# sergcpp/Ray

Hardware: AMD Instinct MI355X
Metric: Msamples/sec (W*H*spp/time) (higher is better)
Workload: dtype f32

## Files before the change

ray_amd/csrc/kernels.hip.h:

```cpp
#pragma once

#include <hip/hip_runtime.h>

#ifdef RT_PROFILE_TRACE
namespace rt {
__device__ unsigned long long g_prof_acc[32];
__shared__ unsigned long long s_prof_last;
__shared__ unsigned long long s_prof_acc[32];
__device__ __forceinline__ void prof_mark(const int k) {
    const unsigned long long mask = __ballot(1);
    if (int(__lane_id()) == __ffsll((long long)mask) - 1) {
        const unsigned long long t = __builtin_readcyclecounter();
        s_prof_acc[k] += t - s_prof_last;
        s_prof_last = t;
    }
}
__device__ __forceinline__ void prof_wait(float4 &a, float4 &b, float4 &c, float4 &d) {
    asm volatile("s_waitcnt vmcnt(0)" : "+v"(a.x), "+v"(b.x), "+v"(c.x), "+v"(d.x));
}
}
#define RT_PROF_T(k) ::rt::prof_mark(k);
#define RT_PROF_LANES(k)                                                                                                \
    {                                                                                                                   \
        const unsigned long long m_ = __ballot(1);                                                                      \
// ... 363 lines not shown
        AccumPixel st = load_accum_pixel(idx, px.full, px.half, px.required_samples);
        const float4 b0 = px.base_color[idx], d0 = px.depth_normals[idx];
        f4 base = {b0.x, b0.y, b0.z, b0.w}, dn = {d0.x, d0.y, d0.z, d0.w};
        AccumParams pl = p;
        for (int k = 0; k < layer_count; ++k) {
            const uint32_t off = layer_offset_xy(layers, uint32_t(layer_base + k));
            const size_t vidx = (size_t(off & 0xffffu) + size_t(y)) * pitch + size_t(off >> 16) + size_t(x);
            fold_layer(pl, per_layer.l[k], px.temp + vidx, px.aux_base_layers + vidx, px.aux_dn_layers + vidx, st, base, dn);
        }
        px.base_color[idx] = mkfloat4(base.x, base.y, base.z, base.w);
        px.depth_normals[idx] = mkfloat4(dn.x, dn.y, dn.z, dn.w);
        store_accum_pixel(pl, idx, st, px.variance + idx, px.full, px.half, px.raw, px.final_, px.required_samples);
    }
}

constexpr int ACCUM_STRIP = 128;
constexpr int ACCUM_SEG_COLS = 8;
constexpr int ACCUM_LOADS = ACCUM_STRIP * ACCUM_SEG_COLS / 256;
static_assert(ACCUM_LOADS * 256 == ACCUM_STRIP * ACCUM_SEG_COLS, "a segment is a whole number of rounds of the block");
__global__ void __launch_bounds__(256) k_accumulate_interleaved(const AccumParams p, const PixelBuffers px, const Layering layers,
                                                               const AccumLayers per_layer, const int layer_base, const int layer_count,
                                                               const int seg_cols) {
    extern __shared__ float4 accum_lds[];
    const int stage = ACCUM_STRIP * seg_cols + 1;
    float4 *const s_temp = accum_lds, *const s_base = accum_lds + stage, *const s_dn = accum_lds + 2 * stage;
    const size_t pitch = size_t(virtual_width(layers));
    const int cols = layers.cols, rows = layers.rows;
    const int strips_x = (p.rect[2] + ACCUM_STRIP - 1) / ACCUM_STRIP, n_strips = strips_x * p.rect[3];
    const int tid = int(threadIdx.x);
    for (int strip = blockIdx.x; strip < n_strips; strip += gridDim.x) {
        const int y = p.rect[1] + strip / strips_x, x0 = p.rect[0] + (strip % strips_x) * ACCUM_STRIP;
        const int np = min(ACCUM_STRIP, p.rect[0] + p.rect[2] - x0);
        const int x = x0 + tid;
        const bool mine = tid < np && pixel_owned(p.shard, p.w, x, y);
        if (!__syncthreads_or(mine ? 1 : 0)) {
            continue;
        }
        const int idx = y * p.w + (mine ? x : x0);
        AccumPixel st = {};
        f4 base = {}, dn = {};
        if (mine) {
            st = load_accum_pixel(idx, px.full, px.half, px.required_samples);
            const float4 b0 = px.base_color[idx], d0 = px.depth_normals[idx];
            base = {b0.x, b0.y, b0.z, b0.w}, dn = {d0.x, d0.y, d0.z, d0.w};
        }
        AccumParams pl = p;
        for (int l0 = layer_base, end = layer_base + layer_count; l0 < end;) {
            const int vr = l0 / cols, c0 = l0 - vr * cols;
            const int len = min(min(seg_cols, cols - c0), end - l0);
            const size_t row0 = (size_t(y) * size_t(rows) + size_t(vr)) * pitch + size_t(x0) * size_t(cols) + size_t(c0);
            const uint32_t rcp = layer_rcp(uint32_t(len));
            const int swizzle = len == 8 ? 7 : 0;
            const int n_elems = np * len;
#pragma unroll
            for (int u = 0; u < ACCUM_LOADS; ++u) {
                const int e = tid + u * 256, e_in = min(e, n_elems - 1);
                const int j = int(div_by_rcp(uint32_t(e_in), rcp));
                const size_t g = row0 + size_t(j) * size_t(cols) + size_t(e_in - j * len);
                const float4 t = px.temp[g], b = px.aux_base_layers[g], d = px.aux_dn_layers[g];
                const int e_out = e < n_elems ? j * len + ((e_in - j * len) ^ (j & swizzle)) : stage - 1;
                s_temp[e_out] = t, s_base[e_out] = b, s_dn[e_out] = d;
            }
            __syncthreads();
            if (mine) {
                for (int k = 0; k < len; ++k) {
                    const int e = tid * len + (k ^ (tid & swizzle));
                    fold_layer(pl, per_layer.l[l0 - layer_base + k], s_temp + e, s_base + e, s_dn + e, st, base, dn);
                }
            }
            __syncthreads();
            l0 += len;
        }
        if (mine) {
            px.base_color[idx] = mkfloat4(base.x, base.y, base.z, base.w);
            px.depth_normals[idx] = mkfloat4(dn.x, dn.y, dn.z, dn.w);
            store_accum_pixel(pl, idx, st, px.variance + idx, px.full, px.half, px.raw, px.final_, px.required_samples);
        }
    }
}

__global__ void __launch_bounds__(256) k_retonemap(const AccumParams p, const PixelBuffers px, const int h) {
    const int n = p.w * h;
    for (int i = blockIdx.x * blockDim.x + threadIdx.x; i < n; i += gridDim.x * blockDim.x) {
        const float4 ff = px.full[i];
        px.raw[i] = ff;
        const f4 c = tonemap(p, f4{ff.x, ff.y, ff.z, ff.w});
// ... 175 lines not shown
```

ray_amd/csrc/rayhip_ctx.hip.h:

```cpp
#pragma once

namespace {
thread_local std::string g_err;

int fail(const char *fmt, ...) {
    char buf[1024];
    va_list vl;
    va_start(vl, fmt);
    vsnprintf(buf, sizeof(buf), fmt, vl);
    va_end(vl);
    g_err = buf;
    return 1;
}

#define HIP_TRY(expr)                                                                                                  \
    do {                                                                                                               \
        const hipError_t _e = (expr);                                                                                  \
        if (_e != hipSuccess) {                                                                                        \
            return fail("%s failed: %s (%s:%d)", #expr, hipGetErrorString(_e), __FILE__, __LINE__);                    \
        }                                                                                                              \
    } while (0)

constexpr int MAX_BOUNCE_SLOTS = 130;

// ... 228 lines not shown
    }
    DevBuf skin_stage;
    DevBuf skin_palettes;
    DevBuf skin_counters;
    DevBuf instance_stage, instance_args, instance_counters;
    bool adaptive_dirty = false;
    int lut_transform = 0, lut_dims = 0;
    PixelBuffers px = {};

    DevBuf ray_planes[2][5], hit_planes[2], shadow_planes[3], deferred_planes[2], point_planes[7], nee_index;
    PointSoA points = {};
    DevBuf pick_plane, record_ray_planes[4];
    RaySoA record_rays = {};
    bool notex_kernels = true;
    bool pick_lds = true;
    bool shade_lds_tables = true;
    uint32_t shade_lds_materials_max = 0xffffffffu, shade_lds_instances_max = 0xffffffffu;
    bool surface_park = true;
    uint32_t shade_tag = 0;
    uint32_t next_shade_tag() {
        if (++shade_tag == 0u) {
            (void)hipMemsetAsync(pick_plane.p, 0, pick_plane.bytes, stream);
            shade_tag = 1u;
        }
        return shade_tag;
    }
    int shade_split = 29;
    RaySoA rays[2] = {};
    HitSoA hits = {};
    ShadowSoA shadow = {};
// ... 483 lines not shown
        c->layer_layout = atoi(e) != 0 ? 1 : 0;
    }
    if (const char *e = getenv("RAYHIP_SORT_KEY")) {
        c->sort_key_mode = std::max(0, std::min(3, atoi(e)));
    }
    if (const char *e = getenv("RAYHIP_SHADE_SPLIT")) {
        c->shade_split = atoi(e) & 31;
        c->shade_form_auto = false;
    }
    if (const char *e = getenv("RAYHIP_NOTEX_KERNELS")) {
        c->notex_kernels = atoi(e) != 0;
    }
    if (const char *e = getenv("RAYHIP_PICK_LDS")) {
        c->pick_lds = atoi(e) != 0;
    }
    if (const char *e = getenv("RAYHIP_SURFACE_PARK")) {
        c->surface_park = atoi(e) != 0;
    }
    if (const char *e = getenv("RAYHIP_SHADE_LDS_TABLES")) {
        c->shade_lds_tables = atoi(e) != 0;
    }
    if (const char *e = getenv("RAYHIP_SHADE_LDS_MATERIALS_MAX")) {
        c->shade_lds_materials_max = uint32_t(std::max(0, atoi(e)));
    }
    if (const char *e = getenv("RAYHIP_SHADE_LDS_INSTANCES_MAX")) {
        c->shade_lds_instances_max = uint32_t(std::max(0, atoi(e)));
    }
    if (c->stack_spill.alloc(size_t(c->grid_waves) * std::max(STACK_SPILL_DEPTH * WAVE, POOL_SLAB_WORDS) * sizeof(uint32_t)) ||
        (c->trace.overlap_shadow && c->stack_spill2.alloc(size_t(c->grid_waves) * size_t(STACK_SPILL_DEPTH * WAVE) * sizeof(uint32_t)))) {
        delete c;
// ... 196 lines not shown
```

ray_amd/csrc/rayhip_render.hip.h:

```cpp
#pragma once

static bool pass_fits(const rayhip_ctx *c, const int rect[4], int n) {
    const Layering L = make_layering(c->w, c->h, n, c->layer_layout);
    const size_t vbytes = size_t(c->w) * size_t(c->h) * size_t(L.cols) * size_t(layer_rows(L)) * 16u;
    return vbytes <= c->px_temp.bytes && (n <= 1 || (vbytes <= c->px_aux_base.bytes && vbytes <= c->px_aux_dn.bytes)) &&
           pass_slots(c, c->w, c->h, rect[2], rect[3], n) + size_t(WAVE) * QUEUE_MAX_STRIPES <= c->slots_cap;
}
static bool rect_inside(const rayhip_ctx *c, const int rect[4]) {
    return rect[0] >= 0 && rect[1] >= 0 && rect[2] > 0 && rect[3] > 0 && rect[0] <= c->w - rect[2] && rect[1] <= c->h - rect[3];
}
static int ensure_pass(rayhip_ctx *c, const int rect[4], int n) {
    if (!rect_inside(c, rect)) {
        return fail("rect outside the frame");
    }
    if (!pass_fits(c, rect, n)) {
        HIP_TRY(hipStreamSynchronize(c->stream));
        if (alloc_frame(c, c->w, c->h, n)) {
            return 1;
        }
    }
    return 0;
}

static void launch_shade(rayhip_ctx *c, const rayhip_camera &cam, int iteration, int bounce, int cur, size_t nslots, uint32_t stripes,
                         int gtrace, int vw, float mix_factor, const Layering &layers, bool plain_ior = false, bool sized = false, int split = -1) {
    ShadeLaunch a;
    a.sc = c->sc;
    a.sp = make_shade_params(cam, iteration, bounce);
    a.sp.plain_ior = plain_ior ? 1u : 0u;
    a.rays_in = c->rays[cur], a.rays_out = c->rays[cur ^ 1];
    a.hits = c->hits, a.shadow = c->shadow, a.deferred = c->deferred, a.points = c->points;
    a.in = c->ray_queue(bounce, nslots, stripes), a.pts = c->point_queue(bounce, nslots, stripes);
    a.out_rays = c->ray_queue(bounce + 1, nslots, stripes), a.out_shadow = c->shadow_queue(bounce, nslots, stripes);
    a.out_deferred = c->deferred_queue(bounce, nslots, stripes), a.nee = c->nee_queue(bounce, nslots, stripes);
    a.out_sky = c->sky_queue(bounce, nslots, stripes), a.sky_index = c->sky_index.as<uint32_t>();
    a.px = c->px, a.layers = layers, a.vw = vw, a.mix_factor = mix_factor;
    a.bounce = bounce, a.grid = gtrace, a.split = split >= 0 ? split : c->shade_split, a.stream = c->stream;
    a.picks = c->pick_plane.as<float4>(), a.record_rays = c->record_rays, a.tag = c->next_shade_tag();
    a.pick_lds = c->pick_lds, a.surface_park = c->surface_park;
    a.lds_tables = c->shade_lds_tables, a.n_materials = c->geometry.materials, a.n_instances = c->instances_count;
    a.lds_materials_max = c->shade_lds_materials_max, a.lds_instances_max = c->shade_lds_instances_max;
    a.no_textures = c->textures_count == 0 && c->notex_kernels;
    if (sized) {
        a.expect[EXPECT_RAYS] = bounce == 0 ? uint32_t(nslots / WAVE + stripes) : c->expect_chunks(bounce, 0, nslots, stripes);
        a.expect[EXPECT_POINTS] = c->expect_chunks(bounce, 3, nslots, stripes), a.expect[EXPECT_LIT] = c->expect_chunks(bounce, 4, nslots, stripes);
        a.expect[EXPECT_DEFERRED] = c->expect_chunks(bounce, 2, nslots, stripes), a.expect[EXPECT_SKY] = c->expect_chunks(bounce, 5, nslots, stripes);
        a.chunks_per_block = c->chunks_per_block;
        a.work = c->next_work(), a.chunks = uint32_t((nslots + WAVE - 1) / WAVE + stripes), a.dyn_mult = c->dyn_mult;
    }
    shade::launch(a);
}

static int render_pass(rayhip_ctx *c, const rayhip_camera *cam, const int rect[4], int iteration, int count_iterations,
                       uint32_t flags, rayhip_stats *stats) {
// ... 38 lines not shown
        return fail("internal: pass of %d iterations exceeds the allocated wavefront state", count_iterations);
    }
    const int gw = c->grid_waves;
    const int gtrace = int(std::min<size_t>(size_t(gw), nslots / WAVE));
    unsigned long long *tc = c->trav_counters.as<unsigned long long>();
    uint32_t *spill = c->stack_spill.as<uint32_t>();
    const TraceParams tp = make_trace_params(*cam, c->sc.tlas_root, iteration);

    const uint32_t stripes = sort_rays ? 1u : QUEUE_MAX_STRIPES;
    if (c->census_on && c->census_pending && hipEventQuery(c->census_event) == hipSuccess) {
        const double inv = c->census_slots ? 1.0 / double(c->census_slots) : 0.0;
        for (int k = 0; k < c->census_bounces * rayhip_ctx::QUEUES_PER_BOUNCE; ++k) {
            c->census[size_t(k)] = float(double(c->census_host[k]) * inv);
        }
        c->census_valid = true, c->census_pending = false;
    }
    int bounce_now = 0;
    auto dyn_grid = [&](int resident, uint32_t expect) {
        const size_t chunks = expect ? size_t(expect) : (nslots + WAVE - 1) / WAVE + stripes;
        return int(std::max<size_t>(1, std::min<size_t>({size_t(gw), size_t(std::max(resident, 1)) * size_t(c->dyn_mult), chunks})));
    };
    auto static_grid = [&](int full, int resident, uint32_t expect) {
        if (!expect) {
            return full;
        }
        const uint32_t want = std::max(std::min(expect, uint32_t(std::max(resident, 1))), expect / uint32_t(c->chunks_per_block));
        return int(std::min<uint32_t>(uint32_t(full), std::max(want, 1u)));
    };
    auto trace_closest = [&](const RaySoA &r, const RayQueue &q, int init_hits) {
        const ClosestForm form = closest_form(c->trace, c->wide, c->direct(), init_hits ? TraceRole::Secondary : TraceRole::Primary, flags);
// ... 145 lines not shown
        side_pending = false;
    }
    if (tm.mark(-1, -1)) {
        return 1;
    }
    AccumParams ap = make_accum_params(*cam, c->w, rect, iteration, c->shard);
    ap.lut = c->tonemap_lut.as<uint32_t>(), ap.lut_dims = c->lut_dims;
    for (int base = 0; base < count_iterations; base += MAX_BATCH) {
        const int n = std::min(MAX_BATCH, count_iterations - base);
        AccumLayers per_layer = {};
        for (int k = 0; k < n; ++k) {
            const AccumParams al = make_accum_params(*cam, c->w, rect, iteration + base + k, c->shard);
            per_layer.l[k] = AccumLayer{al.iteration, al.mix_factor, al.half_mix_factor, al.is_class_a, al.variance_threshold};
        }
        if (layers.interleaved && layers.count > 1) {
            const int seg_cols = std::min(layers.cols, ACCUM_SEG_COLS);
            const size_t strips = size_t((rect[2] + ACCUM_STRIP - 1) / ACCUM_STRIP) * size_t(rect[3]);
            const size_t lds = 3u * (size_t(ACCUM_STRIP) * size_t(seg_cols) + 1u) * sizeof(float4);
            k_accumulate_interleaved<<<grid_for(c, strips * 256u, 256), 256, lds, s>>>(ap, c->px, layers, per_layer, base, n, seg_cols);
        } else {
            k_accumulate<<<grid_for(c, npix, 256), 256, 0, s>>>(ap, c->px, layers, per_layer, base, n);
        }
    }
    if (c->census_on && !count && !count_wide) {
        const int queues = (max_depth + 1) * rayhip_ctx::QUEUES_PER_BOUNCE;
        k_queue_totals<<<queues, WAVE, 0, s>>>(c->counters.as<uint32_t>(), c->census_dev);
        HIP_TRY(hipEventRecord(c->census_event, s));
        c->census_pending = true, c->census_bounces = max_depth + 1, c->census_slots = nslots;
    }
    HIP_TRY(hipGetLastError());
    if (tm.mark(-1, -1)) {
        return 1;
    }
    if (stats) {
// ... 71 lines not shown
```

ray_amd/csrc/shade_kernels.hip:

```cpp
#include <hip/hip_runtime.h>

#include <algorithm>
#include <map>
#include <mutex>
#include <utility>

#ifdef RT_PROFILE_SHADE
namespace rt {
__device__ unsigned long long g_prof_shade[64];
}
#define RT_PROF_SHADE_LANES(k)                                                                                          \
    {                                                                                                                   \
        const unsigned long long m_ = __ballot(1);                                                                      \
        if (int(__lane_id()) == __ffsll((long long)m_) - 1) {                                                           \
            atomicAdd(&::rt::g_prof_shade[k], (unsigned long long)__popcll(m_));                                        \
            atomicAdd(&::rt::g_prof_shade[(k) + 1], 1ull);                                                              \
        }                                                                                                               \
    }
#endif

#include "shade_launch.h"

namespace rt {
namespace shade {
// ... 586 lines not shown
        }
        Scatter sct;
        sct.has_next = sct.has_shadow = false;
        if (continues) {
            ray.o = pt.P, ray.pdf = 0.0f;
            scatter_stage<false, true>(sc, tb, spl, ray, pt, no_light_pick(), sct, &ahead);
            sct.next.xy = xy;
        }
        const uint32_t n_slot = out_rays.alloc(stripe, sct.has_next);
        if (sct.has_next) {
            store_ray(rays_out, n_slot, sct.next, sp.plain_ior == 0u);
        }
    }
}

__global__ void __launch_bounds__(WAVE) k_shade_emissive(const SceneView sc, const ShadeParams sp, const RaySoA rays_in, const HitSoA hits,
                                                        const DeferredSoA deferred, const RayQueue queue, const PixelBuffers px,
                                                        const int img_w) {
    const uint32_t lane = threadIdx.x;
    const uint32_t n_live_chunks = queue.live_chunks();
    ChunkWalk walk(n_live_chunks);
    for (uint32_t c; walk.next(c);) {
        uint32_t stripe, slot0, n_live;
        if (!queue.chunk(c, stripe, slot0, n_live) || lane >= n_live) {
            continue;
        }
        const float4 a = deferred.a[slot0 + lane], b = deferred.b[slot0 + lane];
        const uint32_t i = float_as_uint(a.x), tri = float_as_uint(a.y), material = float_as_uint(a.z);
        const float4 o = rays_in.o_pdf[i], d = rays_in.d_cw[i], throughput = rays_in.c_cs[i];
        const uint32_t xy = rays_in.xy_depth[i].x;
        const Hit hit = load_hit(hits, i);
        const f3 origin = {o.x, o.y, o.z}, dir = {d.x, d.y, d.z};
        const float mis = emissive_hit_mis_weight(sc, origin, dir, origin + hit.t * dir, hit.t, o.w, tri, &sc.mesh_instances[hit.obj_index]);
        ShadeResult res;
        res.col = emissive_hit_radiance(sp, a.w, mis, sc.materials[material].tangent_rotation_or_strength, f3{b.x, b.y, b.z},
                                        f3{throughput.x, throughput.y, throughput.z});
        add_secondary_pixel(res, xy, img_w, px.temp);
    }
}
// ... 9 lines not shown
        if (!queue.chunk(c, stripe, slot0, n_live) || lane >= n_live) {
            continue;
        }
        const uint32_t i = sky_index[slot0 + lane];
        Ray ray = load_ray(rays_in, i, sp.plain_ior == 0u);
        const Hit hit = load_hit(hits, i);
        const uint32_t xy = ray.xy, layer = xy_layer(xy, layers);
        const ShadeParams spl = layer_params(sp, layer);
        ray.xy = xy_real(xy, layers, layer);
        add_sky_pixel(shade_sky_ray(sc, ray, hit, spl.iteration, int(spl.ps.max_total_depth), spl.limits[0]), xy, img_w, px.temp);
    }
}



static int resident_blocks(const void *kernel) {
    static std::mutex mu;
    static std::map<std::pair<int, const void *>, int> cache;
    int dev = 0;
    (void)hipGetDevice(&dev);
    std::lock_guard<std::mutex> lock(mu);
    const auto key = std::make_pair(dev, kernel);
    const auto it = cache.find(key);
    if (it != cache.end()) {
        return it->second;
    }
    int per_cu = 0, cus = 0;
    if (hipOccupancyMaxActiveBlocksPerMultiprocessor(&per_cu, kernel, WAVE, 0) != hipSuccess || per_cu <= 0 ||
        hipDeviceGetAttribute(&cus, hipDeviceAttributeMultiprocessorCount, dev) != hipSuccess) {
        per_cu = 0;
    }
    return cache[key] = per_cu * cus;
}

void launch(const ShadeLaunch &a) {
    hipStream_t s = a.stream;
    const int g = a.grid;
    auto sized = [&](auto kernel, const uint32_t expect, const int cap) {
        int grid = std::min(g, cap);
        if (expect != 0u && a.chunks_per_block > 0) {
            const int resident = std::max(1, resident_blocks(reinterpret_cast<const void *>(kernel)));
            const uint32_t want = std::max(std::min(expect, uint32_t(resident)), expect / uint32_t(a.chunks_per_block));
            grid = int(std::min<uint32_t>(uint32_t(grid), std::max(want, 1u)));
        }
        return grid;
    };
    const int all = 1 << 30;
    if ((a.split & 16) != 0) {
        const bool lights = a.sc.light_cwnodes_count != 0;
        if (lights) {
            const uint32_t lds_nodes = (a.pick_lds && a.sc.light_cwnodes_count <= PICK_LDS_MAX_NODES) ? a.sc.light_cwnodes_count : 0u;
            auto go = [&](auto kernel, auto kernel_wave) {
                int grid = sized(kernel_wave, a.expect[EXPECT_RAYS], all);
                if (a.work) {
                    const int resident = std::max(1, resident_blocks(reinterpret_cast<const void *>(kernel_wave))) * std::max(1, a.dyn_mult);
                    const uint32_t bound = a.expect[EXPECT_RAYS] != 0u ? a.expect[EXPECT_RAYS] : a.chunks;
                    grid = int(std::max<uint32_t>(1u, std::min<uint32_t>({uint32_t(g), uint32_t(resident), std::max(bound, 1u)})));
                }
                if (lds_nodes != 0u) {
                    kernel<<<(grid + PICK_BLOCK_WAVES - 1) / PICK_BLOCK_WAVES, PICK_BLOCK_WAVES * WAVE, size_t(lds_nodes) * LIGHT_CHILDREN_STRIDE * sizeof(float4), s>>>(
                        a.sc, a.sp, a.rays_in, a.hits, a.in, a.picks, a.tag, a.layers, a.work, lds_nodes);
                } else {
                    kernel_wave<<<grid, WAVE, 0, s>>>(a.sc, a.sp, a.rays_in, a.hits, a.in, a.picks, a.tag, a.layers, a.work, 0u);
                }
            };
            a.work ? go(k_light_pick_first<true, true>, k_light_pick_first<true, false>) : go(k_light_pick_first<false, true>, k_light_pick_first<false, false>);
        }
#define RT_FUSED(...) k_surface_scatter<__VA_ARGS__><<<sized(k_surface_scatter<__VA_ARGS__>, a.expect[EXPECT_RAYS], all), WAVE, 0, s>>>( \
        a.sc, a.sp, a.rays_in, a.hits, a.in, a.picks, a.tag, a.points, a.record_rays, a.nee, a.rays_out, a.out_rays, a.deferred, a.out_deferred, a.px, a.vw, \
        a.mix_factor, a.layers, a.sky_index, a.out_sky, a.n_materials, a.n_instances)
// ... 15 lines not shown
        } else if (sky_scene) {
            RT_FUSED(false, true);
        } else if (a.no_textures) {
            if (lds_tables) {
                park ? RT_FUSED(false, false, false, true, true) : RT_FUSED(false, false, false, false, true);
            } else {
                park ? RT_FUSED(false, false, false, true) : RT_FUSED(false, false, false);
            }
        } else {
            RT_FUSED(false, false);
        }
#undef RT_FUSED
        if (sky_scene) {
            k_shade_sky<<<sized(k_shade_sky, a.expect[EXPECT_SKY], 4096), WAVE, 0, s>>>(a.sc, a.sp, a.rays_in, a.hits, a.sky_index, a.out_sky, a.px, a.vw, a.layers);
        }
        k_shade_emissive<<<sized(k_shade_emissive, a.expect[EXPECT_DEFERRED], 2048), WAVE, 0, s>>>(a.sc, a.sp, a.rays_in, a.hits, a.deferred, a.out_deferred, a.px, a.vw);
        if (lights) {
            auto nee = [&](auto kernel) {
                kernel<<<sized(kernel, a.expect[EXPECT_LIT], all), WAVE, 0, s>>>(
                    a.sc, a.sp, a.record_rays, a.points, a.nee, a.rays_out, a.out_rays, a.shadow, a.out_shadow, a.px, a.vw, a.layers, a.pts, a.nee, a.n_materials);
            };
            (lds_tables && a.no_textures) ? nee(k_scatter<true, false, false, 0, true>) : nee(k_scatter<true, false>);
        }
        return;
    }
    const bool pick_apart = (a.split & 1) != 0 && a.sc.light_cwnodes_count != 0;
#define RT_SURFACE_ARGS a.sc, a.sp, a.rays_in, a.hits, a.in, a.points, a.pts, a.deferred, a.out_deferred, a.px, a.vw, a.mix_factor, a.layers, a.sky_index, a.out_sky
#define RT_SURFACE(...) k_surface<__VA_ARGS__><<<sized(k_surface<__VA_ARGS__>, a.expect[EXPECT_RAYS], all), WAVE, 0, s>>>(RT_SURFACE_ARGS)
    const bool sky = a.sc.sky.desc != nullptr;
    if (a.bounce == 0) {
        if (sky) {
// ... 13 lines not shown
                RT_SURFACE(false, false, true);
            } else {
                RT_SURFACE(false, true, true);
            }
        } else if (pick_apart) {
            RT_SURFACE(false, false);
        } else {
            RT_SURFACE(false, true);
        }
    }
#undef RT_SURFACE
#undef RT_SURFACE_ARGS
    if (a.sc.sky.desc != nullptr) {
        k_shade_sky<<<sized(k_shade_sky, a.expect[EXPECT_SKY], 4096), WAVE, 0, s>>>(a.sc, a.sp, a.rays_in, a.hits, a.sky_index, a.out_sky, a.px, a.vw, a.layers);
    }
    k_shade_emissive<<<sized(k_shade_emissive, a.expect[EXPECT_DEFERRED], 2048), WAVE, 0, s>>>(a.sc, a.sp, a.rays_in, a.hits, a.deferred, a.out_deferred, a.px, a.vw);
    const bool nee_compact = pick_apart && (a.split & 4) != 0;
    const bool pick_refill = (a.split & 8) != 0;
    if (pick_apart && pick_refill) {
        auto go = [&](auto kernel) {
            int grid = sized(kernel, a.expect[EXPECT_POINTS], all);
            if (a.work) {
                const int resident = std::max(1, resident_blocks(reinterpret_cast<const void *>(kernel))) * std::max(1, a.dyn_mult);
                const uint32_t bound = a.expect[EXPECT_POINTS] != 0u ? a.expect[EXPECT_POINTS] : a.chunks;
                grid = int(std::max<uint32_t>(1u, std::min<uint32_t>({uint32_t(g), uint32_t(resident), std::max(bound, 1u)})));
            }
            kernel<<<grid, WAVE, 0, s>>>(a.sc, a.sp, a.rays_in, a.points, a.pts, a.nee, a.layers, a.work);
        };
        if (a.work) {
            nee_compact ? go(k_light_pick_refill<true, true>) : go(k_light_pick_refill<false, true>);
        } else {
// ... 39 lines not shown
```

ray_amd/csrc/shade_launch.h:

```cpp
#pragma once

#include "rt_shade.h"
#include "wavefront.hip.h"

namespace rt {

struct PointSoA {
    float4 *p_slot;
    float4 *n_gx;
    float4 *b_gy;
    float4 *base_gz;
    float4 *scalars;
    float4 *misc;
    float4 *light;
    uint32_t *nee_index;
};

struct ShadeLaunch {
    SceneView sc;
    ShadeParams sp;
    RaySoA rays_in, rays_out;
    HitSoA hits;
    ShadowSoA shadow;
    DeferredSoA deferred;
    PointSoA points;
    RayQueue in, pts, out_rays, out_shadow, out_deferred, nee, out_sky;
    uint32_t *sky_index;
    PixelBuffers px;
    Layering layers;
    int vw;
    float mix_factor;
    int bounce, grid;
    uint32_t expect[5] = {0, 0, 0, 0, 0};
    int chunks_per_block = 0;
    uint32_t *work = nullptr;
    uint32_t chunks = 0;
    int dyn_mult = 1;
    bool no_textures = false;
    bool pick_lds = true;
    bool surface_park = true;
    bool lds_tables = true;
    uint32_t n_materials = 0, n_instances = 0;
    uint32_t lds_materials_max = 0xffffffffu, lds_instances_max = 0xffffffffu;
    float4 *picks = nullptr;
    uint32_t tag = 0;
    RaySoA record_rays = {};
    int split;
    hipStream_t stream;
};
enum { EXPECT_RAYS = 0, EXPECT_POINTS, EXPECT_LIT, EXPECT_DEFERRED, EXPECT_SKY };
namespace shade {
void launch(const ShadeLaunch &a);
}

// ... 2 lines not shown
```

ray_amd/csrc/shade_lights.h:

```cpp
#pragma once

#include "rt_rng.h"
#include "rt_texture.h"
#include "rt_types.h"

namespace rt {

struct LightSample {
    f3 radiance;
    f3 dir;
    f3 point;
    float area;
    float reach;
    float pdf;
    bool casts_shadow, is_env;
    uint32_t ray_mask;
};
RT_HD LightSample no_light_sample() {
    LightSample s;
    s.radiance = s.dir = s.point = f3{0.0f, 0.0f, 0.0f};
    s.area = 0.0f, s.reach = 1.0f, s.pdf = 0.0f;
    s.casts_shadow = false, s.is_env = false, s.ray_mask = 0;
    return s;
}
// ... 687 lines not shown
    }
    s.pdf /= pick.inv_prob;
    return s;
}

RT_HD uint32_t children_containing(const rayhip_light_cwbvh_node &n, const f3 p) {
    uint32_t mask = 0;
    for (int i = 0; i < 8; ++i) {
        float lo[3], hi[3];
        light_child_box(n, i, lo, hi);
        const bool inside = (lo[0] <= p.x) && (lo[1] <= p.y) && (lo[2] <= p.z) && (hi[0] >= p.x) && (hi[1] >= p.y) && (hi[2] >= p.z);
        mask |= (inside ? 1u : 0u) << i;
    }
    return mask;
}
RT_HD float triangle_light_inv_pick_prob(const SceneView &sc, const f3 P, const f3 origin, const uint32_t tri) {
    uint32_t todo[MAX_STACK_SIZE];
    float todo_prob[MAX_STACK_SIZE];
    uint32_t n_todo = 0;
    todo_prob[n_todo] = 1.0f;
    todo[n_todo++] = 0;
    while (n_todo) {
        const uint32_t cur = todo[--n_todo];
        const float prob = todo_prob[n_todo];
        if ((cur & LEAF_NODE_BIT) != 0) {
            const rayhip_light &l = sc.lights[cur & PRIM_INDEX_BITS];
            if (light_type(l) == LIGHT_TYPE_TRI && float_as_uint(l.params[0]) == tri) {
                return 1.0f / prob;
            }
            continue;
        }
        const rayhip_light_cwbvh_node &node = sc.light_cwnodes[cur];
        const uint32_t mask = children_containing(node, P);
        if (mask == 0) {
            continue;
        }
        float imp[8];
        light_node_importances(sc, cur, origin, imp);
        const float total = sum8_sse_order(imp);
        if (total == 0.0f) {
            continue;
        }
        for (int i = 0; i < 8; ++i) {
            if (((mask >> i) & 1u) && imp[i] > 0.0f) {
                todo_prob[n_todo] = steer_div(prob * imp[i], total);
                todo[n_todo++] = node.child[i];
            }
        }
    }
    return 1.0f;
}

}
```

ray_amd/csrc/shade_point.h:

```cpp
#pragma once

#include "shade_lights.h"
#include "shade_math.h"

namespace rt {

struct PassLimits {
    int max_diff_depth, max_spec_depth, max_refr_depth, max_transp_depth, max_total_depth;
    int min_total_depth, min_transp_depth;
    float regularize_alpha;
};
struct ShadeParams {
    PassLimits ps;
    float limits[2];
    uint32_t rand_seed;
    int iteration;
    uint32_t plain_ior;
};

struct PathRandom {
    uint32_t hash, dim;
    int sample;
    const uint32_t *table;
    RT_HD f2 get(const int which) const { return get_scrambled_2d_rand(dim + uint32_t(which), hash, sample, table); }
// ... 150 lines not shown
    } break;
    case LIGHT_TYPE_LINE: {
        const float cos_theta = 1.0f - fabsf(dot(ray.d, mk3(&l.params[8])));
        nee_pdf = (hit.t * hit.t) / (l.params[3] * cos_theta * inv_pick_prob);
    } break;
    default:
        weighted = false;
        break;
    }
    if (weighted) {
        c *= power_heuristic(ray.pdf, nee_pdf);
    }
    return c;
}

RT_HD float emissive_hit_mis_weight(const SceneView &sc, const f3 origin, const f3 dir, const f3 P, const float t, const float bsdf_pdf,
                                    const uint32_t tri, const rayhip_mesh_instance *inst) {
    const float inv_pick_prob = triangle_light_inv_pick_prob(sc, P, origin, tri);
    const f3 p1 = mk3(sc.vertices[sc.vtx_indices[tri * 3 + 0]].p), p2 = mk3(sc.vertices[sc.vtx_indices[tri * 3 + 1]].p),
             p3 = mk3(sc.vertices[sc.vtx_indices[tri * 3 + 2]].p);
    float twice_area;
    const f3 facing = normalize_len(transform_direction(cross(p2 - p1, p3 - p1), inst->xform), twice_area);
    const float cos_theta = fabsf(dot(dir, facing));
    if (!(cos_theta > 0.0f)) {
        return 1.0f;
    }
    float nee_pdf = solid_angle_triangle(transform_point(origin, inst->inv_xform), p1, p2, p3, f2{0.0f, 0.0f}, nullptr) / inv_pick_prob;
    if (nee_pdf == 0.0f) {
        nee_pdf = (t * t) / (0.5f * twice_area * cos_theta * inv_pick_prob);
    }
    return power_heuristic(bsdf_pdf, nee_pdf);
}
RT_HD f4 emissive_hit_radiance(const ShadeParams &sp, const float mix_weight, const float mis_weight, const float strength, const f3 base,
                               const f3 throughput) {
    f3 c = {0.0f, 0.0f, 0.0f};
    c += mix_weight * mis_weight * strength * base;
    c *= throughput;
    return mk4(clamp_radiance_sum(c, sp.limits[1]), 1.0f);
}

struct SceneTables {
    const rayhip_material *materials;
    const rayhip_mesh_instance *instances;
    RT_HD const rayhip_material &material(const uint32_t i) const { return materials[i]; }
    RT_HD const float *inv_xform(const uint32_t i) const { return instances[i].inv_xform; }
};
// ... 201 lines not shown
```

Baseline: 802.0.

## Stage light tree in LDS for emissive shading and prefetch accumulation segments

Adds an LDS-tree variant of the emissive-hit shading kernel. It copies light BVH node rows into shared memory per block, keeps a small todo stack in registers that spills to a global overflow buffer, and reads triangle corners from tri_verts. Separately, the interleaved accumulate kernel is templated and software-pipelined so the next segment's global loads are issued before folding the current one. This trades extra LDS and register use plus an up-front tree copy for fewer scattered global reads, and caps the todo stack at MAX_STACK_SIZE.

Measured after the change: 806.5, median of 6. About the same (+0.6%).

```diff
diff --git a/ray_amd/csrc/kernels.hip.h b/ray_amd/csrc/kernels.hip.h
--- a/ray_amd/csrc/kernels.hip.h
+++ b/ray_amd/csrc/kernels.hip.h
@@ -401,23 +401,29 @@
     }
 }
 
-constexpr int ACCUM_STRIP = 128;
-constexpr int ACCUM_SEG_COLS = 8;
-constexpr int ACCUM_LOADS = ACCUM_STRIP * ACCUM_SEG_COLS / 256;
-static_assert(ACCUM_LOADS * 256 == ACCUM_STRIP * ACCUM_SEG_COLS, "a segment is a whole number of rounds of the block");
+constexpr int ACCUM_STRIP = 128, ACCUM_SEG_COLS = 8;
+typedef float accum_vec4 __attribute__((ext_vector_type(4)));
+struct AccumSegment {
+    size_t row0;
+    uint32_t rcp;
+    int len, swizzle, n_elems;
+};
+template <int STRIP, int SEG_COLS>
 __global__ void __launch_bounds__(256) k_accumulate_interleaved(const AccumParams p, const PixelBuffers px, const Layering layers,
                                                                const AccumLayers per_layer, const int layer_base, const int layer_count,
                                                                const int seg_cols) {
+    constexpr int LOADS = STRIP * SEG_COLS / 256;
+    static_assert(LOADS * 256 == STRIP * SEG_COLS && STRIP <= 256, "a segment is a whole number of rounds of the block; a thread folds at most one pixel");
     extern __shared__ float4 accum_lds[];
-    const int stage = ACCUM_STRIP * seg_cols + 1;
+    const int stage = STRIP * seg_cols + 1;
     float4 *const s_temp = accum_lds, *const s_base = accum_lds + stage, *const s_dn = accum_lds + 2 * stage;
     const size_t pitch = size_t(virtual_width(layers));
     const int cols = layers.cols, rows = layers.rows;
-    const int strips_x = (p.rect[2] + ACCUM_STRIP - 1) / ACCUM_STRIP, n_strips = strips_x * p.rect[3];
+    const int strips_x = (p.rect[2] + STRIP - 1) / STRIP, n_strips = strips_x * p.rect[3];
     const int tid = int(threadIdx.x);
     for (int strip = blockIdx.x; strip < n_strips; strip += gridDim.x) {
-        const int y = p.rect[1] + strip / strips_x, x0 = p.rect[0] + (strip % strips_x) * ACCUM_STRIP;
-        const int np = min(ACCUM_STRIP, p.rect[0] + p.rect[2] - x0);
+        const int y = p.rect[1] + strip / strips_x, x0 = p.rect[0] + (strip % strips_x) * STRIP;
+        const int np = min(STRIP, p.rect[0] + p.rect[2] - x0);
         const int x = x0 + tid;
         const bool mine = tid < np && pixel_owned(p.shard, p.w, x, y);
         if (!__syncthreads_or(mine ? 1 : 0)) {
@@ -432,31 +438,57 @@
             base = {b0.x, b0.y, b0.z, b0.w}, dn = {d0.x, d0.y, d0.z, d0.w};
         }
         AccumParams pl = p;
-        for (int l0 = layer_base, end = layer_base + layer_count; l0 < end;) {
+        const int end = layer_base + layer_count;
+        auto segment_at = [&](const int l0) {
             const int vr = l0 / cols, c0 = l0 - vr * cols;
-            const int len = min(min(seg_cols, cols - c0), end - l0);
-            const size_t row0 = (size_t(y) * size_t(rows) + size_t(vr)) * pitch + size_t(x0) * size_t(cols) + size_t(c0);
-            const uint32_t rcp = layer_rcp(uint32_t(len));
-            const int swizzle = len == 8 ? 7 : 0;
-            const int n_elems = np * len;
+            AccumSegment sg;
+            sg.len = min(min(seg_cols, cols - c0), end - l0);
+            sg.row0 = (size_t(y) * size_t(rows) + size_t(vr)) * pitch + size_t(x0) * size_t(cols) + size_t(c0);
+            sg.rcp = layer_rcp(uint32_t(sg.len));
+            sg.swizzle = sg.len == 8 ? 7 : 0;
+            sg.n_elems = np * sg.len;
+            return sg;
+        };
+        accum_vec4 rt[LOADS], rb[LOADS], rd[LOADS];
+        auto fetch = [&](const AccumSegment &sg) {
 #pragma unroll
-            for (int u = 0; u < ACCUM_LOADS; ++u) {
-                const int e = tid + u * 256, e_in = min(e, n_elems - 1);
-                const int j = int(div_by_rcp(uint32_t(e_in), rcp));
-                const size_t g = row0 + size_t(j) * size_t(cols) + size_t(e_in - j * len);
-                const float4 t = px.temp[g], b = px.aux_base_layers[g], d = px.aux_dn_layers[g];
-                const int e_out = e < n_elems ? j * len + ((e_in - j * len) ^ (j & swizzle)) : stage - 1;
-                s_temp[e_out] = t, s_base[e_out] = b, s_dn[e_out] = d;
-            }
+            for (int u = 0; u < LOADS; ++u) {
+                const int e_in = min(tid + u * 256, sg.n_elems - 1);
+                const int j = int(div_by_rcp(uint32_t(e_in), sg.rcp));
+                const size_t g = sg.row0 + size_t(j) * size_t(cols) + size_t(e_in - j * sg.len);
+                rt[u] = *reinterpret_cast<const accum_vec4 *>(px.temp + g), rb[u] = *reinterpret_cast<const accum_vec4 *>(px.aux_base_layers + g);
+                rd[u] = *reinterpret_cast<const accum_vec4 *>(px.aux_dn_layers + g);
+            }
+        };
+        auto stash = [&](const AccumSegment &sg) {
+#pragma unroll
+            for (int u = 0; u < LOADS; ++u) {
+                const int e = tid + u * 256, e_in = min(e, sg.n_elems - 1);
+                const int j = int(div_by_rcp(uint32_t(e_in), sg.rcp));
+                const int e_out = e < sg.n_elems ? j * sg.len + ((e_in - j * sg.len) ^ (j & sg.swizzle)) : stage - 1;
+                *reinterpret_cast<accum_vec4 *>(s_temp + e_out) = rt[u], *reinterpret_cast<accum_vec4 *>(s_base + e_out) = rb[u];
+                *reinterpret_cast<accum_vec4 *>(s_dn + e_out) = rd[u];
+            }
+        };
+        AccumSegment cur = segment_at(layer_base);
+        fetch(cur);
+        for (int l0 = layer_base; l0 < end;) {
+            stash(cur);
             __syncthreads();
+            const int l1 = l0 + cur.len;
+            AccumSegment next = cur;
+            if (l1 < end) {
+                next = segment_at(l1);
+                fetch(next);
+            }
             if (mine) {
-                for (int k = 0; k < len; ++k) {
-                    const int e = tid * len + (k ^ (tid & swizzle));
+                for (int k = 0; k < cur.len; ++k) {
+                    const int e = tid * cur.len + (k ^ (tid & cur.swizzle));
                     fold_layer(pl, per_layer.l[l0 - layer_base + k], s_temp + e, s_base + e, s_dn + e, st, base, dn);
                 }
             }
             __syncthreads();
-            l0 += len;
+            l0 = l1, cur = next;
         }
         if (mine) {
             px.base_color[idx] = mkfloat4(base.x, base.y, base.z, base.w);
diff --git a/ray_amd/csrc/rayhip_ctx.hip.h b/ray_amd/csrc/rayhip_ctx.hip.h
--- a/ray_amd/csrc/rayhip_ctx.hip.h
+++ b/ray_amd/csrc/rayhip_ctx.hip.h
@@ -266,6 +266,7 @@
     RaySoA record_rays = {};
     bool notex_kernels = true;
     bool pick_lds = true;
+    bool emissive_lds = true;
     bool shade_lds_tables = true;
     uint32_t shade_lds_materials_max = 0xffffffffu, shade_lds_instances_max = 0xffffffffu;
     bool surface_park = true;
@@ -779,6 +780,9 @@
     if (const char *e = getenv("RAYHIP_PICK_LDS")) {
         c->pick_lds = atoi(e) != 0;
     }
+    if (const char *e = getenv("RAYHIP_EMISSIVE_LDS")) {
+        c->emissive_lds = atoi(e) != 0;
+    }
     if (const char *e = getenv("RAYHIP_SURFACE_PARK")) {
         c->surface_park = atoi(e) != 0;
     }
diff --git a/ray_amd/csrc/rayhip_render.hip.h b/ray_amd/csrc/rayhip_render.hip.h
--- a/ray_amd/csrc/rayhip_render.hip.h
+++ b/ray_amd/csrc/rayhip_render.hip.h
@@ -38,6 +38,7 @@
     a.bounce = bounce, a.grid = gtrace, a.split = split >= 0 ? split : c->shade_split, a.stream = c->stream;
     a.picks = c->pick_plane.as<float4>(), a.record_rays = c->record_rays, a.tag = c->next_shade_tag();
     a.pick_lds = c->pick_lds, a.surface_park = c->surface_park;
+    a.emissive_lds = c->emissive_lds, a.todo_overflow = c->stack_spill.as<uint32_t>(), a.todo_overflow_words = c->stack_spill.bytes / sizeof(uint32_t);
     a.lds_tables = c->shade_lds_tables, a.n_materials = c->geometry.materials, a.n_instances = c->instances_count;
     a.lds_materials_max = c->shade_lds_materials_max, a.lds_instances_max = c->shade_lds_instances_max;
     a.no_textures = c->textures_count == 0 && c->notex_kernels;
@@ -106,6 +107,13 @@
             c->census[size_t(k)] = float(double(c->census_host[k]) * inv);
         }
         c->census_valid = true, c->census_pending = false;
+        if (getenv("RAYHIP_TRACE_LAUNCH") != nullptr) {
+            fprintf(stderr, "rayhip census (%zu ray slots): deferred emitter hits per bounce", c->census_slots);
+            for (int b = 0; b < c->census_bounces; ++b) {
+                fprintf(stderr, " %u", c->census_host[b * rayhip_ctx::QUEUES_PER_BOUNCE + 2]);
+            }
+            fprintf(stderr, "\n");
+        }
     }
     int bounce_now = 0;
     auto dyn_grid = [&](int resident, uint32_t expect) {
@@ -281,10 +289,13 @@
             per_layer.l[k] = AccumLayer{al.iteration, al.mix_factor, al.half_mix_factor, al.is_class_a, al.variance_threshold};
         }
         if (layers.interleaved && layers.count > 1) {
-            const int seg_cols = std::min(layers.cols, ACCUM_SEG_COLS);
-            const size_t strips = size_t((rect[2] + ACCUM_STRIP - 1) / ACCUM_STRIP) * size_t(rect[3]);
-            const size_t lds = 3u * (size_t(ACCUM_STRIP) * size_t(seg_cols) + 1u) * sizeof(float4);
-            k_accumulate_interleaved<<<grid_for(c, strips * 256u, 256), 256, lds, s>>>(ap, c->px, layers, per_layer, base, n, seg_cols);
+            auto fold = [&](auto kernel, const int strip, const int max_cols) {
+                const int seg_cols = std::min(layers.cols, max_cols);
+                const size_t strips = size_t((rect[2] + strip - 1) / strip) * size_t(rect[3]);
+                const size_t lds = 3u * (size_t(strip) * size_t(seg_cols) + 1u) * sizeof(float4);
+                kernel<<<grid_for(c, strips * 256u, 256), 256, lds, s>>>(ap, c->px, layers, per_layer, base, n, seg_cols);
+            };
+            fold(k_accumulate_interleaved<ACCUM_STRIP, ACCUM_SEG_COLS>, ACCUM_STRIP, ACCUM_SEG_COLS);
         } else {
             k_accumulate<<<grid_for(c, npix, 256), 256, 0, s>>>(ap, c->px, layers, per_layer, base, n);
         }
diff --git a/ray_amd/csrc/shade_kernels.hip b/ray_amd/csrc/shade_kernels.hip
--- a/ray_amd/csrc/shade_kernels.hip
+++ b/ray_amd/csrc/shade_kernels.hip
@@ -3,6 +3,7 @@
 #include <algorithm>
 #include <map>
 #include <mutex>
+#include <tuple>
 #include <utility>
 
 #ifdef RT_PROFILE_SHADE
@@ -624,15 +625,121 @@
     }
 }
 
-__global__ void __launch_bounds__(WAVE) k_shade_emissive(const SceneView sc, const ShadeParams sp, const RaySoA rays_in, const HitSoA hits,
+#ifndef RT_EMISSIVE_LDS_MIN_WAVES
+#define RT_EMISSIVE_LDS_MIN_WAVES 5
+#endif
+constexpr int EMISSIVE_TODO_REGS = 4;
+constexpr uint32_t EMISSIVE_OVERFLOW_WORDS = uint32_t(MAX_STACK_SIZE - EMISSIVE_TODO_REGS) * 2u * uint32_t(WAVE);
+constexpr uint32_t EMISSIVE_LDS_MAX_NODES = (160u * 1024u / (32u / uint32_t(PICK_BLOCK_WAVES)) - 2048u) / (uint32_t(LIGHT_WALK_STRIDE) * 16u);
+struct EmissiveTree : LightTreeRows {
+    __device__ __forceinline__ uint32_t containing(const uint32_t node, const f3 p) const {
+        const rayhip_light_cwbvh_node &n = *reinterpret_cast<const rayhip_light_cwbvh_node *>(node_rows(node) + LIGHT_CHILDREN_STRIDE);
+        uint32_t mask = 0;
+#pragma unroll 1
+        for (int i = 0; i < 8; ++i) {
+            float lo[3], hi[3];
+            light_child_box(n, i, lo, hi);
+            const bool inside = (lo[0] <= p.x) && (lo[1] <= p.y) && (lo[2] <= p.z) && (hi[0] >= p.x) && (hi[1] >= p.y) && (hi[2] >= p.z);
+            mask |= (inside ? 1u : 0u) << i;
+        }
+        return mask;
+    }
+};
+struct EmissiveTodo {
+    uint32_t node[EMISSIVE_TODO_REGS];
+    float prob[EMISSIVE_TODO_REGS];
+    uint32_t *over;
+    __device__ __forceinline__ uint32_t *entry(const uint32_t slot) const {
+        uint32_t l = __lane_id();
+        asm volatile("" : "+v"(l));
+        return over + (slot - uint32_t(EMISSIVE_TODO_REGS)) * uint32_t(2 * WAVE) + l;
+    }
+    __device__ __forceinline__ void put(const uint32_t slot, const uint32_t n, const float p) {
+        if (slot < uint32_t(EMISSIVE_TODO_REGS)) {
+#pragma unroll
+            for (int k = 0; k < EMISSIVE_TODO_REGS; ++k) {
+                node[k] = slot == uint32_t(k) ? n : node[k];
+                prob[k] = slot == uint32_t(k) ? p : prob[k];
+            }
+        } else {
+            uint32_t *e = entry(slot);
+            e[0] = n, e[WAVE] = float_as_uint(p);
+        }
+    }
+    __device__ __forceinline__ void get(const uint32_t slot, uint32_t &n, float &p) const {
+        if (slot < uint32_t(EMISSIVE_TODO_REGS)) {
+            n = node[0], p = prob[0];
+#pragma unroll
+            for (int k = 1; k < EMISSIVE_TODO_REGS; ++k) {
+                n = slot == uint32_t(k) ? node[k] : n;
+                p = slot == uint32_t(k) ? prob[k] : p;
+            }
+        } else {
+            const volatile uint32_t *e = entry(slot);
+            n = e[0], p = uint_as_float(e[WAVE]);
+        }
+    }
+};
+template <bool LDS_TREE>
+__global__ void __launch_bounds__(LDS_TREE ? PICK_BLOCK_WAVES *WAVE : WAVE, LDS_TREE ? RT_EMISSIVE_LDS_MIN_WAVES : 1) k_shade_emissive(const SceneView sc, const ShadeParams sp, const RaySoA rays_in, const HitSoA hits,
                                                         const DeferredSoA deferred, const RayQueue queue, const PixelBuffers px,
-                                                        const int img_w) {
-    const uint32_t lane = threadIdx.x;
+                                                        const int img_w, const uint32_t lds_nodes, uint32_t *__restrict__ todo_overflow) {
+    extern __shared__ float4 s_walk[];
+    const uint32_t lane = LDS_TREE ? (threadIdx.x & uint32_t(WAVE - 1)) : threadIdx.x;
+    const uint32_t waves = LDS_TREE ? uint32_t(PICK_BLOCK_WAVES) : 1u;
+    const uint32_t wave = blockIdx.x * waves + (LDS_TREE ? threadIdx.x / WAVE : 0u);
     const uint32_t n_live_chunks = queue.live_chunks();
-    ChunkWalk walk(n_live_chunks);
+    if (LDS_TREE) {
+        if (blockIdx.x * waves >= n_live_chunks) {
+            return;
+        }
+        for (uint32_t e = threadIdx.x; e < lds_nodes * uint32_t(LIGHT_WALK_STRIDE); e += blockDim.x) {
+            const uint32_t node = e / uint32_t(LIGHT_WALK_STRIDE), r = e - node * uint32_t(LIGHT_WALK_STRIDE);
+            s_walk[e] = r < uint32_t(LIGHT_CHILDREN_STRIDE) ? sc.light_children[size_t(node) * LIGHT_CHILDREN_STRIDE + r]
+                                                            : reinterpret_cast<const float4 *>(sc.light_cwnodes + node)[r - uint32_t(LIGHT_CHILDREN_STRIDE)];
+        }
+        __syncthreads();
+    }
+    ChunkWalk walk(n_live_chunks, nullptr, 1u, wave, gridDim.x * waves);
     for (uint32_t c; walk.next(c);) {
         uint32_t stripe, slot0, n_live;
         if (!queue.chunk(c, stripe, slot0, n_live) || lane >= n_live) {
+            continue;
+        }
+        if constexpr (LDS_TREE) {
+            uint32_t slot = slot0 + lane;
+            float inv_pick_prob;
+            {
+                const float4 a = deferred.a[slot];
+                const uint32_t i = float_as_uint(a.x);
+                const float4 o = rays_in.o_pdf[i], d = rays_in.d_cw[i];
+                const f3 origin = {o.x, o.y, o.z};
+                EmissiveTodo todo;
+#pragma unroll
+                for (int k = 0; k < EMISSIVE_TODO_REGS; ++k) {
+                    todo.node[k] = 0u, todo.prob[k] = 0.0f;
+                }
+                todo.over = todo_overflow + size_t(wave) * size_t(EMISSIVE_OVERFLOW_WORDS);
+                inv_pick_prob = triangle_light_inv_pick_prob_walk(sc, EmissiveTree{{s_walk}}, todo, origin + load_hit(hits, i).t * f3{d.x, d.y, d.z}, origin,
+                                                                  float_as_uint(a.y));
+            }
+            park_fence();
+            asm volatile("" : "+v"(slot));
+            const float4 a = deferred.a[slot];
+            uint32_t i = float_as_uint(a.x);
+            const float4 o = rays_in.o_pdf[i], d = rays_in.d_cw[i];
+            const Hit hit = load_hit(hits, i);
+            const float4 *rows = sc.tri_verts + size_t(float_as_uint(a.y)) * TRI_VERTS_STRIDE;
+            const float4 c1 = rows[0], c2 = rows[2], c3 = rows[4];
+            const float mis = emissive_hit_mis_weight_corners(inv_pick_prob, f3{c1.x, c1.y, c1.z}, f3{c2.x, c2.y, c2.z}, f3{c3.x, c3.y, c3.z}, f3{o.x, o.y, o.z},
+                                                              f3{d.x, d.y, d.z}, hit.t, o.w, &sc.mesh_instances[hit.obj_index]);
+            park_fence();
+            asm volatile("" : "+v"(slot), "+v"(i));
+            const float4 b = deferred.b[slot], throughput = rays_in.c_cs[i];
+            ShadeResult res;
+            res.col = emissive_hit_radiance(sp, a.w, mis, sc.materials[float_as_uint(a.z)].tangent_rotation_or_strength, f3{b.x, b.y, b.z},
+                                            f3{throughput.x, throughput.y, throughput.z});
+            add_secondary_pixel(res, rays_in.xy_depth[i].x, img_w, px.temp);
             continue;
         }
         const float4 a = deferred.a[slot0 + lane], b = deferred.b[slot0 + lane];
@@ -672,19 +779,19 @@
 
 
 
-static int resident_blocks(const void *kernel) {
+static int resident_blocks(const void *kernel, const int threads = WAVE, const size_t lds_bytes = 0) {
     static std::mutex mu;
-    static std::map<std::pair<int, const void *>, int> cache;
+    static std::map<std::tuple<int, const void *, int, size_t>, int> cache;
     int dev = 0;
     (void)hipGetDevice(&dev);
     std::lock_guard<std::mutex> lock(mu);
-    const auto key = std::make_pair(dev, kernel);
+    const auto key = std::make_tuple(dev, kernel, threads, lds_bytes);
     const auto it = cache.find(key);
     if (it != cache.end()) {
         return it->second;
     }
     int per_cu = 0, cus = 0;
-    if (hipOccupancyMaxActiveBlocksPerMultiprocessor(&per_cu, kernel, WAVE, 0) != hipSuccess || per_cu <= 0 ||
+    if (hipOccupancyMaxActiveBlocksPerMultiprocessor(&per_cu, kernel, threads, lds_bytes) != hipSuccess || per_cu <= 0 ||
         hipDeviceGetAttribute(&cus, hipDeviceAttributeMultiprocessorCount, dev) != hipSuccess) {
         per_cu = 0;
     }
@@ -694,24 +801,42 @@
 void launch(const ShadeLaunch &a) {
     hipStream_t s = a.stream;
     const int g = a.grid;
-    auto sized = [&](auto kernel, const uint32_t expect, const int cap) {
+    auto sized = [&](auto kernel, const uint32_t expect, const int cap, const int held = 0) {
         int grid = std::min(g, cap);
         if (expect != 0u && a.chunks_per_block > 0) {
-            const int resident = std::max(1, resident_blocks(reinterpret_cast<const void *>(kernel)));
+            const int resident = std::max(1, held > 0 ? held : resident_blocks(reinterpret_cast<const void *>(kernel)));
             const uint32_t want = std::max(std::min(expect, uint32_t(resident)), expect / uint32_t(a.chunks_per_block));
             grid = int(std::min<uint32_t>(uint32_t(grid), std::max(want, 1u)));
         }
         return grid;
     };
     const int all = 1 << 30;
+    auto launch_emissive = [&]() {
+        const int grid = sized(k_shade_emissive<false>, a.expect[EXPECT_DEFERRED], 2048);
+        const size_t slab_blocks = a.todo_overflow ? a.todo_overflow_words / (size_t(EMISSIVE_OVERFLOW_WORDS) * PICK_BLOCK_WAVES) : 0u;
+        if (a.emissive_lds && a.sc.light_cwnodes_count != 0u && a.sc.light_cwnodes_count <= EMISSIVE_LDS_MAX_NODES && slab_blocks != 0u) {
+            const size_t lds_bytes = size_t(a.sc.light_cwnodes_count) * LIGHT_WALK_STRIDE * sizeof(float4);
+            const int held = resident_blocks(reinterpret_cast<const void *>(k_shade_emissive<true>), PICK_BLOCK_WAVES * WAVE, lds_bytes) * PICK_BLOCK_WAVES;
+            const int waves = a.expect[EXPECT_DEFERRED] != 0u ? sized(k_shade_emissive<true>, a.expect[EXPECT_DEFERRED], all, held) : grid;
+            const int blocks = int(std::min<size_t>(size_t((waves + PICK_BLOCK_WAVES - 1) / PICK_BLOCK_WAVES), slab_blocks));
+            k_shade_emissive<true><<<blocks, PICK_BLOCK_WAVES * WAVE, size_t(a.sc.light_cwnodes_count) * LIGHT_WALK_STRIDE * sizeof(float4), s>>>(
+                a.sc, a.sp, a.rays_in, a.hits, a.deferred, a.out_deferred, a.px, a.vw, a.sc.light_cwnodes_count, a.todo_overflow);
+        } else {
+            k_shade_emissive<false><<<grid, WAVE, 0, s>>>(a.sc, a.sp, a.rays_in, a.hits, a.deferred, a.out_deferred, a.px, a.vw, 0u, nullptr);
+        }
+    };
     if ((a.split & 16) != 0) {
         const bool lights = a.sc.light_cwnodes_count != 0;
         if (lights) {
             const uint32_t lds_nodes = (a.pick_lds && a.sc.light_cwnodes_count <= PICK_LDS_MAX_NODES) ? a.sc.light_cwnodes_count : 0u;
             auto go = [&](auto kernel, auto kernel_wave) {
-                int grid = sized(kernel_wave, a.expect[EXPECT_RAYS], all);
+                const size_t lds_bytes = size_t(lds_nodes) * LIGHT_CHILDREN_STRIDE * sizeof(float4);
+                const int held = lds_nodes != 0u
+                                     ? resident_blocks(reinterpret_cast<const void *>(kernel), PICK_BLOCK_WAVES * WAVE, lds_bytes) * PICK_BLOCK_WAVES
+                                     : resident_blocks(reinterpret_cast<const void *>(kernel_wave));
+                int grid = sized(kernel_wave, a.expect[EXPECT_RAYS], all, held);
                 if (a.work) {
-                    const int resident = std::max(1, resident_blocks(reinterpret_cast<const void *>(kernel_wave))) * std::max(1, a.dyn_mult);
+                    const int resident = std::max(1, held) * std::max(1, a.dyn_mult);
                     const uint32_t bound = a.expect[EXPECT_RAYS] != 0u ? a.expect[EXPECT_RAYS] : a.chunks;
                     grid = int(std::max<uint32_t>(1u, std::min<uint32_t>({uint32_t(g), uint32_t(resident), std::max(bound, 1u)})));
                 }
@@ -757,7 +882,7 @@
         if (sky_scene) {
             k_shade_sky<<<sized(k_shade_sky, a.expect[EXPECT_SKY], 4096), WAVE, 0, s>>>(a.sc, a.sp, a.rays_in, a.hits, a.sky_index, a.out_sky, a.px, a.vw, a.layers);
         }
-        k_shade_emissive<<<sized(k_shade_emissive, a.expect[EXPECT_DEFERRED], 2048), WAVE, 0, s>>>(a.sc, a.sp, a.rays_in, a.hits, a.deferred, a.out_deferred, a.px, a.vw);
+        launch_emissive();
         if (lights) {
             auto nee = [&](auto kernel) {
                 kernel<<<sized(kernel, a.expect[EXPECT_LIT], all), WAVE, 0, s>>>(
@@ -801,7 +926,7 @@
     if (a.sc.sky.desc != nullptr) {
         k_shade_sky<<<sized(k_shade_sky, a.expect[EXPECT_SKY], 4096), WAVE, 0, s>>>(a.sc, a.sp, a.rays_in, a.hits, a.sky_index, a.out_sky, a.px, a.vw, a.layers);
     }
-    k_shade_emissive<<<sized(k_shade_emissive, a.expect[EXPECT_DEFERRED], 2048), WAVE, 0, s>>>(a.sc, a.sp, a.rays_in, a.hits, a.deferred, a.out_deferred, a.px, a.vw);
+    launch_emissive();
     const bool nee_compact = pick_apart && (a.split & 4) != 0;
     const bool pick_refill = (a.split & 8) != 0;
     if (pick_apart && pick_refill) {
diff --git a/ray_amd/csrc/shade_launch.h b/ray_amd/csrc/shade_launch.h
--- a/ray_amd/csrc/shade_launch.h
+++ b/ray_amd/csrc/shade_launch.h
@@ -38,6 +38,9 @@
     int dyn_mult = 1;
     bool no_textures = false;
     bool pick_lds = true;
+    bool emissive_lds = true;
+    uint32_t *todo_overflow = nullptr;
+    size_t todo_overflow_words = 0;
     bool surface_park = true;
     bool lds_tables = true;
     uint32_t n_materials = 0, n_instances = 0;
diff --git a/ray_amd/csrc/shade_lights.h b/ray_amd/csrc/shade_lights.h
--- a/ray_amd/csrc/shade_lights.h
+++ b/ray_amd/csrc/shade_lights.h
@@ -1,4 +1,6 @@
 #pragma once
+
+#include <cstddef>
 
 #include "rt_rng.h"
 #include "rt_texture.h"
@@ -725,15 +727,39 @@
     }
     return mask;
 }
-RT_HD float triangle_light_inv_pick_prob(const SceneView &sc, const f3 P, const f3 origin, const uint32_t tri) {
-    uint32_t todo[MAX_STACK_SIZE];
-    float todo_prob[MAX_STACK_SIZE];
+constexpr int LIGHT_NODE_HEAD_ROWS = 5;
+static_assert(offsetof(rayhip_light_cwbvh_node, child) == size_t(LIGHT_NODE_HEAD_ROWS) * 16u && sizeof(rayhip_light_cwbvh_node) % 16u == 0u,
+              "the node's boxes are its first five float4 rows, and nodes are whole rows");
+struct LightTreeMemory {
+    const SceneView &sc;
+    RT_HD uint32_t containing(const uint32_t node, const f3 p) const { return children_containing(sc.light_cwnodes[node], p); }
+    RT_HD void importances(const uint32_t node, const f3 origin, float imp[8]) const { light_node_importances(sc, node, origin, imp); }
+    RT_HD uint32_t link(const uint32_t node, const int i) const { return sc.light_cwnodes[node].child[i]; }
+};
+constexpr int LIGHT_WALK_STRIDE = LIGHT_CHILDREN_STRIDE + LIGHT_NODE_HEAD_ROWS;
+struct LightTreeRows {
+    const float4 *rows;
+    RT_HD const float4 *node_rows(const uint32_t node) const { return rows + node * uint32_t(LIGHT_WALK_STRIDE); }
+    RT_HD uint32_t containing(const uint32_t node, const f3 p) const {
+        return children_containing(*reinterpret_cast<const rayhip_light_cwbvh_node *>(node_rows(node) + LIGHT_CHILDREN_STRIDE), p);
+    }
+    RT_HD void importances(const uint32_t node, const f3 origin, float imp[8]) const { light_node_importances_rows(node_rows(node), origin, imp); }
+    RT_HD uint32_t link(const uint32_t node, const int i) const { return light_child_link_rows(node_rows(node), i); }
+};
+struct LightTodoArrays {
+    uint32_t node[MAX_STACK_SIZE];
+    float prob[MAX_STACK_SIZE];
+    RT_HD void put(const uint32_t slot, const uint32_t n, const float p) { node[slot] = n, prob[slot] = p; }
+    RT_HD void get(const uint32_t slot, uint32_t &n, float &p) const { n = node[slot], p = prob[slot]; }
+};
+template <class Tree, class Todo>
+RT_HD float triangle_light_inv_pick_prob_walk(const SceneView &sc, const Tree &tree, Todo &todo, const f3 P, const f3 origin, const uint32_t tri) {
     uint32_t n_todo = 0;
-    todo_prob[n_todo] = 1.0f;
-    todo[n_todo++] = 0;
+    todo.put(n_todo++, 0u, 1.0f);
     while (n_todo) {
-        const uint32_t cur = todo[--n_todo];
-        const float prob = todo_prob[n_todo];
+        uint32_t cur;
+        float prob;
+        todo.get(--n_todo, cur, prob);
         if ((cur & LEAF_NODE_BIT) != 0) {
             const rayhip_light &l = sc.lights[cur & PRIM_INDEX_BITS];
             if (light_type(l) == LIGHT_TYPE_TRI && float_as_uint(l.params[0]) == tri) {
@@ -741,25 +767,27 @@
             }
             continue;
         }
-        const rayhip_light_cwbvh_node &node = sc.light_cwnodes[cur];
-        const uint32_t mask = children_containing(node, P);
+        const uint32_t mask = tree.containing(cur, P);
         if (mask == 0) {
             continue;
         }
         float imp[8];
-        light_node_importances(sc, cur, origin, imp);
+        tree.importances(cur, origin, imp);
         const float total = sum8_sse_order(imp);
         if (total == 0.0f) {
             continue;
         }
         for (int i = 0; i < 8; ++i) {
-            if (((mask >> i) & 1u) && imp[i] > 0.0f) {
-                todo_prob[n_todo] = steer_div(prob * imp[i], total);
-                todo[n_todo++] = node.child[i];
+            if (((mask >> i) & 1u) && imp[i] > 0.0f && n_todo < uint32_t(MAX_STACK_SIZE)) {
+                todo.put(n_todo++, tree.link(cur, i), steer_div(prob * imp[i], total));
             }
         }
     }
     return 1.0f;
 }
-
-}
+RT_HD float triangle_light_inv_pick_prob(const SceneView &sc, const f3 P, const f3 origin, const uint32_t tri) {
+    LightTodoArrays todo;
+    return triangle_light_inv_pick_prob_walk(sc, LightTreeMemory{sc}, todo, P, origin, tri);
+}
+
+}
diff --git a/ray_amd/csrc/shade_point.h b/ray_amd/csrc/shade_point.h
--- a/ray_amd/csrc/shade_point.h
+++ b/ray_amd/csrc/shade_point.h
@@ -188,22 +188,26 @@
     return c;
 }
 
+RT_HD float emissive_hit_mis_weight_corners(const float inv_pick_prob, const f3 p1, const f3 p2, const f3 p3, const f3 origin, const f3 dir,
+                                            const float t, const float bsdf_pdf, const rayhip_mesh_instance *inst) {
+    float twice_area;
+    const f3 facing = normalize_len(transform_direction(cross(p2 - p1, p3 - p1), inst->xform), twice_area);
+    const float cos_theta = fabsf(dot(dir, facing));
+    if (!(cos_theta > 0.0f)) {
+        return 1.0f;
+    }
+    float nee_pdf = solid_angle_triangle(transform_point(origin, inst->inv_xform), p1, p2, p3, f2{0.0f, 0.0f}, nullptr) / inv_pick_prob;
+    if (nee_pdf == 0.0f) {
+        nee_pdf = (t * t) / (0.5f * twice_area * cos_theta * inv_pick_prob);
+    }
+    return power_heuristic(bsdf_pdf, nee_pdf);
+}
 RT_HD float emissive_hit_mis_weight(const SceneView &sc, const f3 origin, const f3 dir, const f3 P, const float t, const float bsdf_pdf,
                                     const uint32_t tri, const rayhip_mesh_instance *inst) {
     const float inv_pick_prob = triangle_light_inv_pick_prob(sc, P, origin, tri);
     const f3 p1 = mk3(sc.vertices[sc.vtx_indices[tri * 3 + 0]].p), p2 = mk3(sc.vertices[sc.vtx_indices[tri * 3 + 1]].p),
              p3 = mk3(sc.vertices[sc.vtx_indices[tri * 3 + 2]].p);
-    float twice_area;
-    const f3 facing = normalize_len(transform_direction(cross(p2 - p1, p3 - p1), inst->xform), twice_area);
-    const float cos_theta = fabsf(dot(dir, facing));
-    if (!(cos_theta > 0.0f)) {
-        return 1.0f;
-    }
-    float nee_pdf = solid_angle_triangle(transform_point(origin, inst->inv_xform), p1, p2, p3, f2{0.0f, 0.0f}, nullptr) / inv_pick_prob;
-    if (nee_pdf == 0.0f) {
-        nee_pdf = (t * t) / (0.5f * twice_area * cos_theta * inv_pick_prob);
-    }
-    return power_heuristic(bsdf_pdf, nee_pdf);
+    return emissive_hit_mis_weight_corners(inv_pick_prob, p1, p2, p3, origin, dir, t, bsdf_pdf, inst);
 }
 RT_HD f4 emissive_hit_radiance(const ShadeParams &sp, const float mix_weight, const float mis_weight, const float strength, const f3 base,
                                const f3 throughput) {
```
